# LanaSina/evolutionary_illusion_generator

Measured on AMD Instinct MI355X. Metric: genome fitness evals/sec at 256x256, pop=256, higher is better.
Workload: dtype f32; 1 GPU; neat_configs/circles.txt colour pop=256, 256x256, PredNet 3,48,96,192, 21 steps, LK + rotation-symmetry score; global_pop=256, genomes_per_gpu=256, device_batch=256, structure=Circles

## Files before the change

### evolutionary_illusion_generator_amd/csrc/conv_wino4.h

```cpp
#pragma once
#include "wino_launch.h"

namespace eig {

constexpr int W4_UPOS = 256;
constexpr int W4_U_FLOATS = W4_NPOS * W4_UPOS;
constexpr int W4_NUS = 3, W4_NPS = 3;
constexpr int w4_row(bool tall) { return tall ? 28 : 40; }
constexpr int w4_ps(bool tall) { return tall ? 1024 : 768; }
constexpr int w4_pslot(bool tall) { return W4_KC * w4_ps(tall); }
constexpr int w4_p(bool tall, int k) { return tall ? k * w4_pslot(true) : (k < 2 ? k * w4_pslot(false) : 2 * w4_pslot(false) + 3 * W4_U_FLOATS); }
constexpr int w4_u(bool tall, int k) { return tall ? 3 * w4_pslot(true) + k * W4_U_FLOATS : 2 * w4_pslot(false) + k * W4_U_FLOATS; }
constexpr int w4_x(bool tall) { return tall ? w4_u(true, 0) : w4_u(false, 1); }
constexpr int W4_X_FLOATS = W4_WAVES * 2 * 4 * 64 * 4;
constexpr int wino4_lds_bytes() { return (w4_x(false) + W4_X_FLOATS) * 4; }
static_assert((w4_u(true, 2) + W4_U_FLOATS) * 4 == wino4_lds_bytes() && (w4_p(false, 2) + w4_pslot(false)) * 4 <= wino4_lds_bytes(), "LDS maps");
#ifndef EIG_W4_DEEPU
#define EIG_W4_DEEPU 1
#endif
#ifndef EIG_W4_DIAG
#define EIG_W4_DIAG 0
#endif

__device__ __forceinline__ void w4_in1d(float d0, float d1, float d2, float d3, float d4, float d5, float* T)
{
    T[0] = fmaf(4.0f, d0, fmaf(-5.0f, d2, d4));
    const float p = fmaf(-4.0f, d2, d4), q = fmaf(-4.0f, d1, d3);
    T[1] = p + q; T[2] = p - q;
    const float r = d4 - d2, s = d3 - d1;
    T[3] = fmaf(2.0f, s, r); T[4] = fmaf(-2.0f, s, r);
    T[5] = fmaf(4.0f, d1, fmaf(-5.0f, d3, d5));
}
template <int XI> __device__ __forceinline__ float w4_row(const float* d)
{
    if constexpr (XI == 0) return fmaf(4.0f, d[0], fmaf(-5.0f, d[1], d[2]));
    else if constexpr (XI == 5) return fmaf(4.0f, d[0], fmaf(-5.0f, d[1], d[2]));
    else {
        if constexpr (XI == 1) return fmaf(-4.0f, d[1], d[3]) + fmaf(-4.0f, d[0], d[2]);
        else if constexpr (XI == 2) return fmaf(-4.0f, d[1], d[3]) - fmaf(-4.0f, d[0], d[2]);
        else if constexpr (XI == 3) return fmaf(2.0f, d[2] - d[0], d[3] - d[1]);
        else return fmaf(-2.0f, d[2] - d[0], d[3] - d[1]);
    }
}
constexpr int w4_nrows(int xi) { return (xi == 0 || xi == 5) ? 3 : 4; }
constexpr int w4_rowidx(int xi, int k) { return xi == 0 ? 2 * k : xi == 5 ? 2 * k + 1 : k + 1; }
constexpr int w4_uprow(int i) { return (i + 1) >> 1; }

template <typename V4> __device__ __forceinline__ void w4_out1d(const V4& m0, const V4& m1, const V4& m2, const V4& m3, const V4& m4, const V4& m5, V4* Y)
{
    const V4 s = m1 + m2, d = m1 - m2, u = m3 + m4, w = m3 - m4;
    Y[0] = (m0 + s) + u;
    for (int e = 0; e < 4; ++e) { Y[1][e] = fmaf(2.0f, w[e], d[e]); Y[2][e] = fmaf(4.0f, u[e], s[e]); Y[3][e] = fmaf(8.0f, w[e], d[e]) + m5[e]; }
}

template <int NI, int EPI, bool TALL = false, bool HALF = false, bool PACK = false, bool NSPLIT = false>
__global__ void __launch_bounds__((HALF && !NSPLIT) ? W4_THREADS / 2 : W4_THREADS, 3) wino4_kernel(const ConvArgs a)
{
    static_assert(!NSPLIT || (HALF && NI == 4 && EPI != EPI_CONVA), "N-split: a half block, 64-column N-blocks, ConvLSTM / ConvP");
    constexpr int NIW = NSPLIT ? 2 : NI;
    constexpr bool DEEPU = HALF && EIG_W4_DEEPU;
    static_assert(!(TALL && HALF), "half blocks exist in the wide shape only");
    static_assert(!PACK || (HALF && EPI != EPI_CONVA), "packed tiles: a half block, ConvLSTM / ConvP");
    constexpr bool TGEO = TALL || PACK;
    static_assert(EPI == EPI_LSTM || EPI == EPI_CONVA || EPI == EPI_CONVP, "conv_wino4.h: ConvLSTM, ConvA, ConvP");
    static_assert(EPI != EPI_LSTM || NI == 4, "ConvLSTM: the four N-tiles are the four gates");
    static_assert(NI == 3 || NI == 4, "N-blocks of 48 or 64 columns");
    constexpr int U4 = wino4_u_floats(NI);
    constexpr int KC = W4_KC, PS = w4_ps(TGEO), W4_ROW = w4_row(TGEO);
    constexpr int W4_P0 = w4_p(TGEO, 0), W4_P1 = w4_p(TGEO, 1), W4_P2 = w4_p(TGEO, 2), W4_U0 = w4_u(TGEO, 0), W4_U1 = w4_u(TGEO, 1), W4_U2 = w4_u(TGEO, 2);
    constexpr int PK_ROWS = 18, PK_CX = 7, PK_IMG = PK_ROWS * PK_CX;
    constexpr bool WALK = !TALL && !HALF;
    constexpr int RGH = TALL ? 16 : 8;
    extern __shared__ __attribute__((aligned(16))) float lds[];
    unsigned long long tq_entry = EIG_TIMING ? __builtin_readcyclecounter() : 0;
    float* const Pb = lds;
    float* const Ub = lds;
    float* const xb = lds + w4_x(TGEO);
    const int wv_o = __builtin_amdgcn_readfirstlane((int)threadIdx.x >> 6);
    const int rg_o = HALF ? 0 : wv_o & 1, xi_o = (HALF && !NSPLIT) ? wv_o : wv_o >> 1;
    const int ng_o = NSPLIT ? wv_o & 1 : 0;
    constexpr int NWAVES = (HALF && !NSPLIT) ? W4_WAVES / 2 : W4_WAVES;
    constexpr int UPW = 36 / NWAVES;
    auto lane_id = [&]() __attribute__((always_inline)) { int l = (int)__builtin_amdgcn_mbcnt_hi(~0u, __builtin_amdgcn_mbcnt_lo(~0u, 0u)); asm volatile("" : "+v"(l)); return l; };

    const int tiles = a.tilesX * a.tilesY;
    const bool pk5 = PACK && a.tilesX == 5;
    const int ntile = PACK ? a.B + (pk5 ? (a.B + 3) >> 2 : 0) : a.B * tiles;
    const int xcd = blockIdx.x & 7, xi_ = blockIdx.x >> 3;
    auto dv = [&](int x, int d, unsigned m) __attribute__((always_inline)) { return m ? (int)__umulhi((unsigned)x, m) : x / d; };
    const int q0 = dv(xi_, a.nparts, a.mg[0]);
    const int part = xi_ - q0 * a.nparts;
    const int tlin = a.tile_map ? xcd * ((ntile + 7) >> 3) + q0 : q0 * 8 + xcd;
    if (tlin >= ntile) return;
    const int nwalk = WALK ? a.nwalk : 1, nb0 = part * nwalk;
    const bool pk_edge_o = pk5 && tlin >= a.B;
    const int eb = PACK ? (pk_edge_o ? 4 * (tlin - a.B) : tlin) : dv(tlin, tiles, a.mg[1]);
    const int t_ = PACK ? 0 : tlin - eb * tiles;
    const int tyi = dv(t_, a.tilesX, a.mg[2]), txi = t_ - tyi * a.tilesX;
    const int y0 = PACK ? 0 : tyi * (TALL ? 32 : (HALF ? 8 : 16)), x0 = PACK ? 0 : txi * (TALL ? 16 : 32);
    const int HW = a.H * a.W;

    const bool up_fused = !PACK && EPI == EPI_LSTM && a.up_src != nullptr;
    const int nkb0 = a.src[0].C / KC;
    const int nkbu = up_fused ? (a.up_C / KC) : 0;
    const bool has1 = a.nsrc > 1;
    const int nkb_o = nkb0 + nkbu + (has1 ? (a.src[1].C / KC) : 0);
    const int up_lo_o = nkb0, up_hi_o = nkb0 + nkbu;
#define EIG4_WAITCNT(imm) do { __builtin_amdgcn_s_waitcnt(imm); asm volatile("" ::: "memory"); } while (0)
#define EIG4_BARRIER() do { asm volatile("" ::: "memory"); __builtin_amdgcn_s_barrier(); asm volatile("" ::: "memory"); } while (0)
#define EIG4_LDS_BARRIER() do { EIG4_WAITCNT(0xC07F); EIG4_BARRIER(); } while (0)
#define EIG4_IS_UP(kb) ((kb) >= up_lo && (kb) < up_hi)

    typedef float f32x2 __attribute__((ext_vector_type(2)));
    constexpr unsigned W4_POSB = 4 * 16 * NI * 4;
    auto walk_body = [&](const int it) __attribute__((always_inline)) {
    const int nblk = nb0 + it;
    int zs = 0;
    asm volatile("" : "+s"(zs));
    const int wv = wv_o + zs, rg = rg_o + zs, xi = xi_o + zs, ng = ng_o + zs, nkb = nkb_o + zs, up_lo = up_lo_o + zs, up_hi = up_hi_o + zs;
    const int pch = HALF ? wv >> 1 : wv / 3, ppart = HALF ? wv & 1 : wv - pch * 3;
    const bool has_plane = !(NSPLIT && !PACK) || wv_o < 8;
    const int eb_i = eb + zs, y0_i = y0 + zs, x0_i = x0 + zs;
    const bool pk_edge = (pk_edge_o ? 1 : 0) + zs != 0;
    const unsigned long long sb0 = (unsigned long long)(a.src[0].ptr + (size_t)eb_i * a.src[0].Ct * HW);
    const unsigned long long sb1 = has1 ? (unsigned long long)(a.src[1].ptr + (size_t)eb_i * a.src[1].Ct * HW) : sb0;
    const int ist0 = a.src[0].Ct * HW * 4, ist1 = has1 ? a.src[1].Ct * HW * 4 : ist0;
    const int sz0 = a.src[0].C * HW * 4 + (PACK ? 3 * ist0 : 0), sz1 = has1 ? a.src[1].C * HW * 4 + (PACK ? 3 * ist1 : 0) : sz0;
    const int Hh = a.H >> 1, Wh = a.W >> 1, HWh = Hh * Wh;
    const unsigned long long sbu = up_fused ? (unsigned long long)(a.up_src + (size_t)eb_i * a.up_C * HWh) : sb0;
    const int szu = up_fused ? a.up_C * HWh * 4 : sz0;
    const int lane = lane_id();
    const int q = lane >> 4, col = lane & 15;
    constexpr int CPR = TALL ? 7 : 10, CREAL = TALL ? 6 : 10, NCHK = TALL ? 34 * 7 : (HALF ? 100 : 180), UROWS = TALL ? 18 : (HALF ? 6 : 10), UCHK = TALL ? 4 : 6;
    auto plane_offsets = [&](int part, int& ro, int& uo) __attribute__((always_inline)) {
        const int c = lane + 64 * part;
        const int row = c / CPR, cx = c - row * CPR;
        const int gy = y0_i - 1 + row, gx = x0_i - 4 + 4 * cx;
        ro = (c < NCHK && cx < CREAL && gy >= 0 && gy < a.H && gx >= 0 && gx < a.W) ? (gy * a.W + gx) * 4 : -1;
        const int hy = (y0_i >> 1) - 1 + row, hx = (x0_i >> 1) - 4 + 4 * cx;
        uo = (row < UROWS && cx < UCHK && hy >= 0 && hy < Hh && hx >= 0 && hx < Wh) ? (hy * Wh + hx) * 4 : -1;
    };
    int pk_ro[3] = {-1, -1, -1};
    unsigned pk_mul[3] = {0u, 0u, 0u};
    const int pk_n = (wv_o < 4 ? 2 : 1) + (NSPLIT ? 0 : 1);
    if constexpr (PACK) {
#pragma unroll
        for (int k = 0; k < 3; ++k) {
            const int c = lane + 64 * ((wv_o + NWAVES * k) & 3);
            const int p = c >= PK_IMG ? 1 : 0, c1 = c - PK_IMG * p;
            const int row = c1 / PK_CX, slot = c1 - row * PK_CX;
            const int b = slot >= 3 ? (slot >= 6 ? 2 : 1) : 0;
            const int irel = pk_edge ? 2 * p + b : 0, cx = pk_edge ? 4 + slot - 3 * b : slot;
            const int gy = row - 1, gx = 4 * cx - 4;
            const bool ok = (pk_edge ? (c < 2 * PK_IMG && b < 2) : c < PK_IMG) && eb_i + irel < a.B && gy >= 0 && gy < a.H && gx >= 0 && gx < a.W;
            pk_ro[k] = ok ? (gy * a.W + gx) * 4 : -1;
            pk_mul[k] = ok ? (unsigned)irel : 0u;
        }
    }
    int roff, uoff, roff2 = -1, uoff2 = -1;
    plane_offsets(ppart, roff, uoff);
    const bool two_parts = (TALL && wv_o < 4) || (HALF && !PACK && !NSPLIT && wv_o < 2);
    if (TALL) plane_offsets(3, roff2, uoff2);
    if (HALF) { roff2 = roff; uoff2 = uoff; }
    const int ch2 = HALF ? 3 : wv, part2 = HALF ? ppart : 3;
    auto dma_plane_at = [&](int jj, int slot_off) __attribute__((always_inline)) {
        const int j = jj < nkb ? jj : nkb - 1;
        const bool up = EIG4_IS_UP(j);
        const bool s1 = j >= up_hi;
        const unsigned long long mu = 0ull - (unsigned long long)up, m1 = 0ull - (unsigned long long)s1;
        const unsigned long long u = sb0 + ((sb1 - sb0) & m1) + ((sbu - sb0) & mu);
        const unsigned lo = __builtin_amdgcn_readfirstlane((unsigned)u), hi = __builtin_amdgcn_readfirstlane((unsigned)(u >> 32));
        const int sz = sz0 + ((sz1 - sz0) & (int)m1) + ((szu - sz0) & (int)mu);
        const __amdgpu_buffer_rsrc_t rs = __builtin_amdgcn_make_buffer_rsrc((void*)(((unsigned long long)hi << 32) | lo), 0, __builtin_amdgcn_readfirstlane(sz), 0x00020000);
        const int base = (up_lo & (int)mu) + (up_hi & (int)m1), hw = HW + ((HWh - HW) & (int)mu);
        if constexpr (PACK) {
            const unsigned ist = (unsigned)(ist0 + ((ist1 - ist0) & (int)m1));
#pragma unroll
            for (int k = 0; k < 3; ++k) {
                if (k >= pk_n) break;
                const int idx = wv_o + NWAVES * k;
                const unsigned coffk = (unsigned)((j - base) * KC + (idx >> 2)) * (unsigned)(hw * 4);
                __builtin_amdgcn_raw_ptr_buffer_load_lds(rs, (__attribute__((address_space(3))) void*)(Pb + slot_off + (idx >> 2) * PS + (idx & 3) * 256), 16,
                                                         (int)__builtin_elementwise_add_sat((unsigned)pk_ro[k] + pk_mul[k] * ist, coffk), 0, 0, 0);
            }
            return;
        }
        if (!has_plane) return;
        const unsigned coff = (unsigned)((j - base) * KC + pch) * (unsigned)(hw * 4);
        __builtin_amdgcn_raw_ptr_buffer_load_lds(rs, (__attribute__((address_space(3))) void*)(Pb + slot_off + pch * PS + ppart * 256), 16,
                                                 (int)__builtin_elementwise_add_sat((unsigned)roff + (((unsigned)uoff - (unsigned)roff) & (unsigned)mu), coff), 0, 0, 0);
        if (two_parts) {
            const unsigned coff2 = (unsigned)((j - base) * KC + ch2) * (unsigned)(hw * 4);
            __builtin_amdgcn_raw_ptr_buffer_load_lds(rs, (__attribute__((address_space(3))) void*)(Pb + slot_off + ch2 * PS + part2 * 256), 16,
                                                     (int)__builtin_elementwise_add_sat((unsigned)roff2 + (((unsigned)uoff2 - (unsigned)roff2) & (unsigned)mu), coff2), 0, 0, 0);
        }
    };
    auto wait_u = [&]() __attribute__((always_inline)) {
        const int npl = PACK ? pk_n : (two_parts ? 2 : (has_plane ? 1 : 0));
        switch (npl + (DEEPU ? UPW : 0)) {
            case 0: EIG4_WAITCNT(0x0F70); break;
            case 1: EIG4_WAITCNT(0x0F71); break;
            case 2: EIG4_WAITCNT(0x0F72); break;
            case 3: EIG4_WAITCNT(0x0F73); break;
            case 4: EIG4_WAITCNT(0x0F74); break;
            case 5: EIG4_WAITCNT(0x0F75); break;
            case 6: EIG4_WAITCNT(0x0F76); break;
            case 7: EIG4_WAITCNT(0x0F77); break;
            case 8: EIG4_WAITCNT(0x0F78); break;
            default: EIG4_WAITCNT(0x0F79); break;
        }
    };
    const int uvo = (NI == 4 || lane < 48) ? lane * 16 : -1;
    auto prologue_a = [&](int nb) __attribute__((always_inline)) {
        const __amdgpu_buffer_rsrc_t rs = __builtin_amdgcn_make_buffer_rsrc((void*)(a.wpk + (size_t)nb * nkb * U4), 0, (nkb + 1) * U4 * 4, 0x00020000);
#pragma unroll
        for (int i = 0; i < UPW; ++i)
            __builtin_amdgcn_raw_ptr_buffer_load_lds(rs, (__attribute__((address_space(3))) void*)(Ub + W4_U0 + (UPW * wv + i) * W4_UPOS), 16, uvo, (int)((unsigned)(UPW * wv + i) * W4_POSB), 0, 0);
        dma_plane_at(0, W4_P0);
        dma_plane_at(1, W4_P1);
    };
    auto prologue_b = [&](int nb) __attribute__((always_inline)) {
        const __amdgpu_buffer_rsrc_t rs = __builtin_amdgcn_make_buffer_rsrc((void*)(a.wpk + (size_t)nb * nkb * U4), 0, (nkb + 1) * U4 * 4, 0x00020000);
#pragma unroll
        for (int i = 0; i < UPW; ++i)
            __builtin_amdgcn_raw_ptr_buffer_load_lds(rs, (__attribute__((address_space(3))) void*)(Ub + W4_U1 + (UPW * wv + i) * W4_UPOS), 16, uvo,
                                                     (int)((unsigned)U4 * 4 + (unsigned)(UPW * wv + i) * W4_POSB), 0, 0);
        dma_plane_at(2, W4_P2);
    };

    const int pk_ir = pk_edge ? col >> 2 : 0, pk_ty = pk_edge ? col & 3 : col >> 2;
    const int t_ty = PACK ? 0 : (TALL ? col >> 2 : col >> 3), t_tx = PACK ? (pk_edge ? 3 * (pk_ir & 1) : col & 3) : (TALL ? col & 3 : col & 7);
    const int pk_row = PACK ? PK_ROWS * (pk_ir >> 1) + 4 * pk_ty : 0;
    const float* const pbase_n = Pb + q * PS + (RGH * rg + 4 * t_ty + pk_row) * W4_ROW + 4 * t_tx;
    const float* const pbase_u = Pb + q * PS + ((RGH / 2) * rg + 2 * t_ty) * W4_ROW + 2 * t_tx + 3;
    const int b_off = xi * 6 * W4_UPOS + (q * 16 + col) * NI + 2 * ng;

    unsigned long long tq_setup = tq_entry;
    if (it == 0) {
        if (EIG_TIMING) tq_setup = __builtin_readcyclecounter();
        prologue_a(nb0);
        EIG4_WAITCNT(0x0F70);
    }
    const __amdgpu_buffer_rsrc_t rsw = __builtin_amdgcn_make_buffer_rsrc((void*)(a.wpk + (size_t)nblk * nkb * U4), 0, (nkb + 1) * U4 * 4, 0x00020000);
    unsigned u_so = (unsigned)(UPW * wv) * W4_POSB + 2u * (unsigned)U4 * 4u;
    auto dma_u = [&](int slot_off) __attribute__((always_inline)) {
#pragma unroll
        for (int i = 0; i < UPW; ++i)
            __builtin_amdgcn_raw_ptr_buffer_load_lds(rsw, (__attribute__((address_space(3))) void*)(Ub + slot_off + (UPW * wv + i) * W4_UPOS), 16, uvo,
                                                     (int)(u_so + (unsigned)i * W4_POSB), 0, 0);
        u_so += (unsigned)U4 * 4;
    };
    f32x4 acc[6][NIW];
#pragma unroll
    for (int p = 0; p < 6; ++p)
#pragma unroll
        for (int ni = 0; ni < NIW; ++ni) acc[p][ni] = (f32x4){0.f, 0.f, 0.f, 0.f};
    EIG4_BARRIER();
    prologue_b(nblk);
    const unsigned long long tq_k0 = EIG_TIMING ? __builtin_readcyclecounter() : 0;
    unsigned long long tq_k1 = 0, tq_x = 0, tq_y = 0;
    auto timeline = [&]() __attribute__((always_inline)) {
        if (EIG_TIMING && a.dbg && lane_id() == 0) {
            unsigned hwid, xcc;
            asm volatile("s_getreg_b32 %0, hwreg(HW_REG_HW_ID)" : "=s"(hwid));
            asm volatile("s_getreg_b32 %0, hwreg(HW_REG_XCC_ID)" : "=s"(xcc));
            unsigned long long* dd = a.dbg + (((size_t)blockIdx.x * nwalk + it) * NWAVES + wv) * 8;
            const unsigned long long tq_end = __builtin_readcyclecounter();
            dd[0] = tq_entry; dd[1] = tq_setup; dd[2] = tq_k0; dd[3] = tq_k1; dd[4] = tq_x; dd[5] = tq_y; dd[6] = tq_end;
            dd[7] = (unsigned long long)hwid | ((unsigned long long)xcc << 32);
            tq_entry = tq_end;
        }
    };

    auto kloops = [&](auto role_tag) __attribute__((always_inline)) {
        constexpr int XI = decltype(role_tag)::value;
        float v[6];
        float bq[NIW];
        int uo0 = W4_U0, uo1 = W4_U1, uo2 = W4_U2;
        int po0 = W4_P0, po1 = W4_P1, po2 = W4_P2;
        int pj = 0, psz = 0, pbound = 0;
// ... 131 lines not shown
                    if constexpr (!FIRST) read_b(uo1, 0, bq);
                    build_cols();
                }
            } else {
#pragma unroll
                for (int i = 0; i < NCH; ++i) {
                    const int nu = (UP && i >= 2) ? i + 1 : i;
                    if (i + 1 < NCH) {
                        const int nu1 = (UP && i + 1 >= 2) ? i + 2 : i + 1;
                        read_b(uo0, nu1, bv[(i + 1) & 1]);
                    } else if constexpr (!LAST && !FIRST) read_b(uo1, 0, bq);
                    const float* const b = i == 0 ? bq : bv[i & 1];
#pragma unroll
                    for (int ni = 0; ni < NIW; ++ni) acc[nu][ni] = __builtin_amdgcn_mfma_f32_16x16x4f32(v[nu], b[ni], acc[nu][ni], 0, 0, 0);
                    slice(i);
                    __builtin_amdgcn_sched_barrier(0);
                }
            }
            { const int t0 = uo0; uo0 = uo1; uo1 = uo2; uo2 = t0; }
            { const int t0 = po0; po0 = po1; po1 = po2; po2 = t0; }
            if (LAST || (EIG_W4_DIAG & (8 | 16))) EIG4_WAITCNT(0x0F70);
            else if (!(EIG_W4_DIAG & 2)) { if (!(EIG_W4_DIAG & 1)) wait_u(); }
            if (!(EIG_W4_DIAG & 2) || LAST) EIG4_BARRIER();
            if constexpr (FIRST) read_b(uo0, 0, bq);
        };
        const std::false_type nl{};
        const std::integral_constant<int, 2> rt{};
        int kb = 0;
        rows_begin(W4_P0, EIG4_IS_UP(0)); rows_mid(); rows_end();
        read_b(W4_U0, 0, bq);
        build_cols();
        EIG4_WAITCNT(0xC07F);
        EIG4_BARRIER();
        auto run = [&](const int end, auto kind_tag) __attribute__((always_inline)) {
            for (; kb + 1 < end; ++kb) kiter(kb, kind_tag, kind_tag, nl, nl);
            if (kb + 1 == end && end < nkb) { kiter(kb, kind_tag, rt, nl, nl); ++kb; }
        };
        kiter(0, std::integral_constant<int, 0>{}, std::integral_constant<int, 0>{}, nl, std::true_type{});
        kb = 1;
        run(up_lo, std::integral_constant<int, 0>{});
        run(up_hi, std::integral_constant<int, 1>{});
        run(nkb, std::integral_constant<int, 0>{});
        kiter(nkb - 1, rt, rt, std::true_type{}, nl);
    };
    switch (xi) {
        case 0: kloops(std::integral_constant<int, 0>{}); break;
        case 1: kloops(std::integral_constant<int, 1>{}); break;
        case 2: kloops(std::integral_constant<int, 2>{}); break;
        case 3: kloops(std::integral_constant<int, 3>{}); break;
        case 4: kloops(std::integral_constant<int, 4>{}); break;
        default: kloops(std::integral_constant<int, 5>{}); break;
    }
    if (EIG_TIMING) tq_k1 = __builtin_readcyclecounter();
    const bool more = it + 1 < nwalk;
    if (more) prologue_a(nblk + 1);

    f32x4 cc[4][NIW];
#pragma unroll
    for (int ni = 0; ni < NIW; ++ni) {
        f32x4 Y[4];
        w4_out1d(acc[0][ni], acc[1][ni], acc[2][ni], acc[3][ni], acc[4][ni], acc[5][ni], Y);
#pragma unroll
        for (int b = 0; b < 4; ++b) cc[b][ni] = Y[b];
    }
    {
    int zf = 0;
    asm volatile("" : "+s"(zf));
    const int eb = eb_i + zf, y0 = y0_i + zf, x0 = x0_i + zf, wv = wv_o + zf, rg = rg_o + zf, xi = xi_o + zf, HWf = HW + zf, Cout = a.Cout + zf, ngf = ng_o + zf;
    const bool pk_edge_f = (pk_edge_o ? 1 : 0) + zf != 0;
    const int lane = lane_id();
    const int q = lane >> 4, col = lane & 15;
    const size_t cHW = (size_t)HWf;
    const int j = TALL ? lane & 3 : lane & 7, chl = TALL ? lane >> 2 : lane >> 3, e_r = j & 3, ql = TALL ? 0 : j >> 2;
    int woff[4];
#pragma unroll
    for (int e = 0; e < 4; ++e) woff[e] = (((2 * xi + (NSPLIT ? ngf : rg)) * 2 * 4 + e) * 64 + q * 16 + ((col + 4 * e + (PACK ? q : (TALL ? 0 : 8 * (q & 1)))) & 15)) * 4;
    const int fr = lane & 15, fchl = lane >> 4;
    const int f_i = pk_edge_f ? fr >> 2 : 0, f_ty = pk_edge_f ? fr & 3 : fr >> 2, f_tx = pk_edge_f ? 4 : fr & 3;
    if constexpr (EPI == EPI_LSTM || EPI == EPI_CONVP) {
        const int nun = NSPLIT ? ((xi < 4 && ngf == 0) ? 2 : 1) : (xi < 4 ? 3 : 2);
        auto unit_cq = [&](int un) __attribute__((always_inline)) { return xi < 4 ? (NSPLIT ? (ngf ? 2 : un) : un) : 3; };
        auto unit_arow = [&](int un) __attribute__((always_inline)) { return xi < 4 ? xi : 2 * (xi - 4) + (NSPLIT ? ngf : un); };
        int xoff[3];
#pragma unroll
        for (int un = 0; un < 3; ++un) {
            const int cq = unit_cq(un);
            const int ty = TALL ? cq : cq >> 1, chh = TALL ? 0 : cq & 1;
            xoff[un] = TALL ? (e_r * 64 + ty * 16 + ((chl + 4 * e_r) & 15)) * 4 : (e_r * 64 + (2 * ty + ql) * 16 + ((8 * chh + chl + 4 * e_r + 8 * ql) & 15)) * 4;
            if constexpr (PACK) xoff[un] = ((fr & 3) * 64 + (fr >> 2) * 16 + ((4 * cq + fchl + 4 * (fr & 3) + (fr >> 2)) & 15)) * 4;
        }
        auto finish = [&](int arow, int nr, int off, int xw) __attribute__((always_inline)) -> f32x4 {
            auto C = [&](int x) __attribute__((always_inline)) { return *reinterpret_cast<const f32x4*>(xb + ((x * 2 + xw) * 2 + nr) * 1024 + off); };
            const f32x4 c1 = C(1), c2 = C(2), c3 = C(3), c4 = C(4);
            const f32x4 s_ = c1 + c2, d_ = c1 - c2, u_ = c3 + c4, w_ = c3 - c4;
            f32x4 y;
            if (arow == 0) { const f32x4 c0 = C(0); y = (c0 + s_) + u_; }
            else if (arow == 1) { for (int b = 0; b < 4; ++b) y[b] = fmaf(2.0f, w_[b], d_[b]); }
            else if (arow == 2) { for (int b = 0; b < 4; ++b) y[b] = fmaf(4.0f, u_[b], s_[b]); }
            else { const f32x4 c5 = C(5); for (int b = 0; b < 4; ++b) y[b] = fmaf(8.0f, w_[b], d_[b]) + c5[b]; }
            return y;
        };
        f32x4 ys[NI][3];
        auto finish_unit = [&](int ni, int nr, int xw, int un) __attribute__((always_inline)) {
            const int sel = NSPLIT ? ngf : un;
            switch (xi) {
                case 0: ys[ni][un] = finish(0, nr, xoff[un], xw); break;
                case 1: ys[ni][un] = finish(1, nr, xoff[un], xw); break;
                case 2: ys[ni][un] = finish(2, nr, xoff[un], xw); break;
                case 3: ys[ni][un] = finish(3, nr, xoff[un], xw); break;
                case 4: ys[ni][un] = sel ? finish(1, nr, xoff[un], xw) : finish(0, nr, xoff[un], xw); break;
                default: ys[ni][un] = sel ? finish(3, nr, xoff[un], xw) : finish(2, nr, xoff[un], xw); break;
            }
        };
        if constexpr (NSPLIT) {
#pragma unroll
            for (int nr = 0; nr < 2; ++nr)
#pragma unroll
                for (int e = 0; e < 4; ++e) {
                    f32x4 t;
                    t[0] = cc[0][nr][e]; t[1] = cc[1][nr][e]; t[2] = cc[2][nr][e]; t[3] = cc[3][nr][e];
                    *reinterpret_cast<f32x4*>(xb + woff[e] + nr * 1024) = t;
                }
            EIG4_LDS_BARRIER();
            if (EIG_TIMING) tq_x = __builtin_readcyclecounter();
#pragma unroll
            for (int ni = 0; ni < NI; ++ni)
#pragma unroll
                for (int un = 0; un < 2; ++un) {
                    if (un >= nun) break;
                    finish_unit(ni, ni & 1, ni >> 1, un);
                }
        } else {
#pragma unroll
        for (int rnd = 0; rnd < 2; ++rnd) {
            if (2 * rnd >= NI) break;
            if (rnd) EIG4_LDS_BARRIER();
#pragma unroll
            for (int nr = 0; nr < 2; ++nr) {
                const int ni = 2 * rnd + nr;
                if (ni >= NI) break;
#pragma unroll
                for (int e = 0; e < 4; ++e) {
                    f32x4 t;
                    t[0] = cc[0][ni][e]; t[1] = cc[1][ni][e]; t[2] = cc[2][ni][e]; t[3] = cc[3][ni][e];
                    *reinterpret_cast<f32x4*>(xb + woff[e] + nr * 1024) = t;
                }
            }
            EIG4_LDS_BARRIER();
            if (EIG_TIMING && rnd == 0) tq_x = __builtin_readcyclecounter();
#pragma unroll
            for (int nr = 0; nr < 2; ++nr) {
                const int ni = 2 * rnd + nr;
                if (ni >= NI) break;
#pragma unroll
                for (int un = 0; un < 3; ++un) {
                    if (un >= nun) break;
                    finish_unit(ni, nr, rg, un);
                }
            }
        }
        }
        if (more) EIG4_WAITCNT(0x0F70);
        if (EIG_TIMING) { asm volatile("s_waitcnt lgkmcnt(0)" ::: "memory"); tq_y = __builtin_readcyclecounter(); }
#pragma unroll
        for (int un = 0; un < 3; ++un) {
            if (un >= nun) break;
            const int cq = unit_cq(un);
            const int ty = TALL ? cq : cq >> 1, chh = TALL ? 0 : cq & 1;
            const int arow = unit_arow(un);
            const int gy = PACK ? 4 * f_ty + arow : y0 + RGH * rg + 4 * ty + arow, gx = PACK ? 4 * f_tx : x0 + 4 * j;
            if (gy >= a.H || gx >= a.W) continue;
            const int ebo = PACK ? eb + f_i : eb;
            if (PACK && ebo >= a.B) continue;
            const size_t pix = (size_t)gy * a.W + gx;
            const int chq = PACK ? 4 * cq + fchl : 8 * chh + chl;
            if constexpr (EPI == EPI_LSTM) {
                const int ch = nblk * 16 + chq;
                if (ch >= Cout) continue;
                const float bi = a.bias[ch], bf = a.bias[Cout + ch], bc = a.bias[2 * Cout + ch], bo = a.bias[3 * Cout + ch];
                const size_t cbase = ((size_t)ebo * Cout + ch) * cHW, ps = (size_t)Cout * cHW, pbase = (size_t)ch * cHW;
                const f32x4 cold4 = *reinterpret_cast<const f32x4*>(a.c_state + cbase + pix);
                const f32x4 pi4 = *reinterpret_cast<const f32x4*>(a.peep + pbase + pix);
                const f32x4 pf4 = *reinterpret_cast<const f32x4*>(a.peep + ps + pbase + pix);
                const f32x4 po4 = *reinterpret_cast<const f32x4*>(a.peep + 2 * ps + pbase + pix);
                f32x4 cn4, hn4;
#pragma unroll
                for (int b = 0; b < 4; ++b) {
                    float cn, hn;
                    lstm_cell(ys[0][un][b], ys[1][un][b], ys[2][un][b], ys[3][un][b], bi, bf, bc, bo, cold4[b], pi4[b], pf4[b], po4[b], cn, hn);
                    cn4[b] = cn; hn4[b] = hn;
                }
                *reinterpret_cast<f32x4*>(a.c_state + cbase + pix) = cn4;
                *reinterpret_cast<f32x4*>(a.h_out + cbase + pix) = hn4;
            } else {
#pragma unroll
                for (int ni = 0; ni < NI; ++ni) {
                    const int ch = (nblk * NI + ni) * 16 + chq;
                    if (ch >= Cout) continue;
                    const float bb_ = a.bias[ch];
                    f32x4 v4;
#pragma unroll
                    for (int b = 0; b < 4; ++b) v4[b] = relu_f(ys[ni][un][b] + bb_);
                    *reinterpret_cast<f32x4*>(a.Pout + ((size_t)ebo * Cout + ch) * cHW + pix) = v4;
                }
            }
        }
    } else {
        const int Ho = a.H >> 1, Wo = a.W >> 1;
        const size_t plane = (size_t)Ho * Wo;
        const int ox = (x0 >> 1) + 2 * j;
#pragma unroll
// ... 10 lines not shown
                    f32x4 t;
                    t[0] = cc[0][ni][e]; t[1] = cc[1][ni][e]; t[2] = cc[2][ni][e]; t[3] = cc[3][ni][e];
                    *reinterpret_cast<f32x4*>(xb + woff[e] + nr * 1024) = t;
                }
            }
            EIG4_LDS_BARRIER();
            if (rnd == (NI - 1) / 2) { if (more) EIG4_WAITCNT(0x0F70); }
            if (EIG_TIMING && rnd == 0) { tq_x = __builtin_readcyclecounter(); tq_y = tq_x; }
            const int g0 = nval == 2 ? (xi < 4 ? 3 * xi : 12 + 2 * (xi - 4)) : (xi < 2 ? 2 * xi : xi + 2);
            const int cnt = nval == 2 ? (xi < 4 ? 3 : 2) : (xi < 2 ? 2 : 1);
#pragma unroll
            for (int un = 0; un < 3; ++un) {
                if (un >= cnt) break;
                const int g = g0 + un;
                const int nr = g >> 3, ty = TALL ? (g >> 1) & 3 : (g >> 2) & 1, ap = TALL ? g & 1 : (g >> 1) & 1, chh = TALL ? 0 : g & 1;
                const int off = TALL ? ((nr + 2 * rg) * 256 + e_r * 64 + ty * 16 + ((chl + 4 * e_r) & 15)) * 4
                                     : ((nr + 2 * rg) * 256 + e_r * 64 + (2 * ty + ql) * 16 + ((8 * chh + chl + 4 * e_r + 8 * ql) & 15)) * 4;
                auto C = [&](int x) __attribute__((always_inline)) { return *reinterpret_cast<const f32x4*>(xb + x * 4096 + off); };
                const f32x4 c1 = C(1), c2 = C(2), c3 = C(3), c4 = C(4);
                const f32x4 s_ = c1 + c2, d_ = c1 - c2, u_ = c3 + c4, w_ = c3 - c4;
                f32x4 ya, yb;
                if (ap == 0) {
                    const f32x4 c0 = C(0);
                    ya = (c0 + s_) + u_;
                    for (int b = 0; b < 4; ++b) yb[b] = fmaf(2.0f, w_[b], d_[b]);
                } else {
                    const f32x4 c5 = C(5);
                    for (int b = 0; b < 4; ++b) { ya[b] = fmaf(4.0f, u_[b], s_[b]); yb[b] = fmaf(8.0f, w_[b], d_[b]) + c5[b]; }
                }
                const int ch = (nblk * NI + 2 * rnd + nr) * 16 + 8 * chh + chl;
                const int oy = (y0 >> 1) + (RGH / 2) * rg + 2 * ty + ap;
                if (oy >= Ho || ox >= Wo || ch >= Cout) continue;
                const float bb_ = a.bias[ch];
                const size_t pb = ((size_t)eb * Cout + ch) * plane + (size_t)oy * Wo + ox;
                const size_t e0 = ((size_t)eb * 2 * Cout + ch) * plane + (size_t)oy * Wo + ox, e1 = e0 + (size_t)Cout * plane;
                const f32x2 p2 = *reinterpret_cast<const f32x2*>(a.P + pb);
                f32x2 ea, eb2;
#pragma unroll
                for (int bp = 0; bp < 2; ++bp) {
                    const float v00 = relu_f(ya[2 * bp] + bb_), v01 = relu_f(ya[2 * bp + 1] + bb_);
                    const float v10 = relu_f(yb[2 * bp] + bb_), v11 = relu_f(yb[2 * bp + 1] + bb_);
                    const float A = fmaxf(fmaxf(v00, v01), fmaxf(v10, v11));
                    ea[bp] = relu_f(A - p2[bp]);
                    eb2[bp] = relu_f(p2[bp] - A);
                }
                *reinterpret_cast<f32x2*>(a.E + e0) = ea;
                *reinterpret_cast<f32x2*>(a.E + e1) = eb2;
            }
        }
    }
    }
    timeline();
    };
    for (int it = 0; it < nwalk; ++it) walk_body(it);
#undef EIG4_WAITCNT
#undef EIG4_BARRIER
#undef EIG4_LDS_BARRIER
#undef EIG4_IS_UP
}

}
```

### evolutionary_illusion_generator_amd/csrc/eigen_engine.hip

```cpp
#include <hip/hip_runtime.h>

#include <algorithm>
#include <cmath>
#include <cstdarg>
#include <cstdio>
#include <cstring>
#include <string>
#include <unordered_map>
#include <unordered_set>
#include <vector>

#include "../../include/eigen_engine.h"
#define EIG_ENGINE_UNIT 1
#include "conv_mfma.h"
#include "wino_launch.h"
#include "cppn_kernel.h"
#include "farneback_kernels.h"
#include "flow_kernels.h"
#include "score_kernels.h"

using namespace eig;

static thread_local std::string g_err;
static int fail(int code, const char* fmt, ...)
// ... 391 lines not shown
    }
}

static hipError_t launch_conv(eigen_engine* e, ConvOp& op, ConvArgs& a, int batch, hipStream_t st)
{
    const int TH = (op.TW == 8) ? 8 : 16;
    const int NIMG = 256 / (TH * op.TW);
    a.H = op.H; a.W = op.W; a.B = batch;
    a.tilesX = (op.W + op.TW - 1) / op.TW;
    a.tilesY = (op.H + TH - 1) / TH;
    a.n_nblk = op.n_nblk; a.krows = op.krows; a.wpk = op.d_wpk; a.Cout = op.Cout; a.zeros = e->d_zeros;
    a.nsrc = op.nsrc;
    for (int s = 0; s < op.nsrc; ++s) { a.src[s].C = op.src_C[s]; a.src[s].Cpad = pad4(op.src_C[s]); a.src[s]._reserved = 0; a.src[s].Ct = op.src_Ct[s] ? op.src_Ct[s] : op.src_C[s]; }
    int ntile = ((batch + NIMG - 1) / NIMG) * a.tilesX * a.tilesY;
    const int per_tile = op.n_nblk * (op.epi == EPI_UP4 ? 4 : 1);
    int grid = per_tile * ((ntile + 7) / 8) * 8;
    const bool vec = (op.W % 4) == 0;
#if EIG_TIMING
    unsigned long long* tl_dbg = nullptr;
    if (getenv("EIGEN_TIMELINE") && (op.epi == EPI_LSTM || (op.epi == EPI_UP4 && op.NI == 4) || (op.wino && getenv("EIGEN_TIMELINE_ALL"))) && ++op.tl_seen == 6) {
        (void)hipMalloc((void**)&tl_dbg, (size_t)grid * 2 * 64 * 8);
        (void)hipMemset(tl_dbg, 0, (size_t)grid * 2 * 64 * 8);
        a.dbg = tl_dbg;
    }
#endif
    {
        static const int tile_map = getenv("EIGEN_TILE_MAP") ? atoi(getenv("EIGEN_TILE_MAP")) : 1;
        a.tile_map = tile_map != 0;
    }
    static const int w8_env = getenv("EIGEN_W8") ? atoi(getenv("EIGEN_W8")) : -1;
    const int w8 = (vec && op.epi == EPI_CONVA && op.TW == 16 && op.NI < 4 && (w8_env >= 0 ? w8_env != 0 : grid <= 8 * e->n_cu)) ? 1 : 0;
    op.last_grid = grid; op.last_waves = (w8 == 1) ? 8 : 4;
    if (e->profile_convs) (void)hipEventRecord(e->pev0, st);
    hipError_t r;
    if (op.wino) {
        if (op.epi == EPI_LSTM && a.acc_init != nullptr) return hipErrorInvalidConfiguration;
        static const int tall_env = getenv("EIGEN_W4_TALL") ? atoi(getenv("EIGEN_W4_TALL")) : -1;
        const bool tall = tall_env >= 0 ? tall_env != 0 : ((op.W + 15) / 16) * ((op.H + 31) / 32) < ((op.W + 31) / 32) * ((op.H + 15) / 16);
        a.tilesX = tall ? (op.W + 15) / 16 : (op.W + 31) / 32; a.tilesY = tall ? (op.H + 31) / 32 : (op.H + 15) / 16;
        static const int half_env = getenv("EIGEN_W4_HALF") ? atoi(getenv("EIGEN_W4_HALF")) : -1;
        const bool half = !tall && (half_env >= 0 ? half_env != 0 : (long long)op.n_nblk * batch * a.tilesX * ((op.H + 7) / 8) <= e->n_cu);
        if (half) a.tilesY = (op.H + 7) / 8;
        static const int pack_env = getenv("EIGEN_W4_PACK") ? atoi(getenv("EIGEN_W4_PACK")) : -1;
        const int ptx = (op.W + 3) / 4, pty = (op.H + 3) / 4;
        const bool pack_can = op.epi != EPI_CONVA && a.up_src == nullptr && (ptx == 4 || ptx == 5) && pty == 4 && tall_env < 0 && half_env < 0;
        bool pack = false;
        if (pack_can) {
            const long long nhalf = (long long)op.n_nblk * (batch + (ptx == 5 ? (batch + 3) / 4 : 0)), nfull = (long long)op.n_nblk * batch;
            pack = pack_env >= 0 ? pack_env != 0 : 2 * ((nhalf + e->n_cu - 1) / e->n_cu) < 3 * ((nfull + e->n_cu - 1) / e->n_cu);
        }
        if (pack) { a.tilesX = ptx; a.tilesY = pty; }
        const int ntile4 = pack ? batch + (ptx == 5 ? (batch + 3) / 4 : 0) : batch * a.tilesX * a.tilesY;
        static const int parts_env = getenv("EIGEN_W4_PARTS") ? atoi(getenv("EIGEN_W4_PARTS")) : 0;
        int nparts;
        if (parts_env > 0) { nparts = std::min(parts_env, op.n_nblk); while (op.n_nblk % nparts) --nparts; }
        else {
            int nwalk = (op.n_nblk % 3 == 0) ? 3 : ((op.n_nblk % 2 == 0) ? 2 : 1);
            if ((long long)(op.n_nblk / nwalk) * ntile4 < 4ll * e->n_cu) nwalk = 1;
            nparts = op.n_nblk / nwalk;
        }
        if (tall || half || pack) nparts = op.n_nblk;
        a.nparts = nparts; a.nwalk = op.n_nblk / nparts;
        const int g4 = nparts * ((ntile4 + 7) / 8) * 8;
        {
            auto magic = [&](long long d) -> unsigned { return (d > 1 && (long long)g4 * 16 * d < (1ll << 32)) ? (unsigned)(((1ll << 32) + d - 1) / d) : 0u; };
            a.mg[0] = magic(nparts); a.mg[1] = magic((long long)a.tilesX * a.tilesY); a.mg[2] = magic(a.tilesX);
        }
        op.last_grid = g4 * a.nwalk; op.last_waves = ((half || pack) && !(op.NI == 4 && op.epi != EPI_CONVA)) ? W4_WAVES / 2 : W4_WAVES;
#if EIG_TIMING
        if (tl_dbg) {
            (void)hipFree(tl_dbg);
            (void)hipMalloc((void**)&tl_dbg, (size_t)op.last_grid * op.last_waves * 64);
            (void)hipMemset(tl_dbg, 0, (size_t)op.last_grid * op.last_waves * 64);
            a.dbg = tl_dbg;
        }
#endif
        r = launch_wino4(op.NI, op.epi, pack ? W4_PACK : (tall ? W4_TALL : (half ? W4_HALF : W4_WIDE)), a, g4, st);
    } else {
    static const bool direct_p0 = !(getenv("EIGEN_CONVP0_MFMA") && atoi(getenv("EIGEN_CONVP0_MFMA")));
    if (op.epi == EPI_CONVP && op.d_wraw && direct_p0) {
        const dim3 g((op.W + P0_TX - 1) / P0_TX, (op.H + P0_TY - 1) / P0_TY, batch);
        if (op.Cout == 3) hipLaunchKernelGGL(convp0_direct_kernel<3>, g, dim3(P0_TX * P0_TY), 0, st, a.src[0].ptr, op.d_wraw, a);
        else hipLaunchKernelGGL(convp0_direct_kernel<1>, g, dim3(P0_TX * P0_TY), 0, st, a.src[0].ptr, op.d_wraw, a);
        r = hipGetLastError();
    } else if (static const bool direct_l0 = !(getenv("EIGEN_LSTM0_MFMA") && atoi(getenv("EIGEN_LSTM0_MFMA")));
               op.epi == EPI_LSTM_PACKED && op.d_wraw && direct_l0 && (op.Cout == 1 || op.Cout == 3)) {
        const dim3 g((op.W + L0_TX - 1) / L0_TX, (op.H + L0_TY - 1) / L0_TY, batch);
        const dim3 blk(L0_TX * L0_TY);
        const float *sE = a.src[0].ptr, *sH = a.src[1].ptr;
        if (op.nsrc == 1) {
            if (op.Cout == 3) hipLaunchKernelGGL((lstm0_direct_kernel<3, true>), g, blk, 0, st, sE, sH, op.d_wraw, a);
            else hipLaunchKernelGGL((lstm0_direct_kernel<1, true>), g, blk, 0, st, sE, sH, op.d_wraw, a);
        } else {
            if (op.Cout == 3) hipLaunchKernelGGL((lstm0_direct_kernel<3, false>), g, blk, 0, st, sE, sH, op.d_wraw, a);
            else hipLaunchKernelGGL((lstm0_direct_kernel<1, false>), g, blk, 0, st, sE, sH, op.d_wraw, a);
        }
        r = hipGetLastError();
    } else
    switch (op.epi) {
        case EPI_LSTM: r = (op.TW == 16) ? launch_inst<4, 16, EPI_LSTM>(a, grid, st, vec) : launch_inst<4, 8, EPI_LSTM>(a, grid, st, vec); break;
        case EPI_LSTM_PACKED: r = (op.TW == 16) ? launch_inst<1, 16, EPI_LSTM_PACKED>(a, grid, st, vec) : launch_inst<1, 8, EPI_LSTM_PACKED>(a, grid, st, vec); break;
        case EPI_CONVA: {
            static const bool onekb = !(getenv("EIGEN_NO_ONEKB") && atoi(getenv("EIGEN_NO_ONEKB")));
            if (onekb && op.NI == 3 && op.TW == 16 && vec && op.nsrc == 1 && pad4(op.src_C[0]) <= KC) r = launch_inst2<3, 16, EPI_CONVA, true, true>(a, grid, st);
            else r = launch_epi<EPI_CONVA>(op.NI, op.TW, a, grid, st, vec, w8);
            break;
        }
        case EPI_CONVP: r = launch_epi<EPI_CONVP>(op.NI, op.TW, a, grid, st, vec, w8); break;
        case EPI_UP4: r = launch_epi<EPI_UP4>(op.NI, op.TW, a, grid, st, vec, w8); break;
        case EPI_UP4C: r = launch_inst2<4, 16, EPI_UP4C, true>(a, grid, st); break;
        default: r = launch_epi<EPI_RAW>(op.NI, op.TW, a, grid, st, vec, w8); break;
    }
    }
#if EIG_TIMING
    if (tl_dbg) {
        (void)hipStreamSynchronize(st);
        std::vector<unsigned long long> h((size_t)op.last_grid * op.last_waves * 8);
        (void)hipMemcpy(h.data(), tl_dbg, h.size() * 8, hipMemcpyDeviceToHost);
        char name[256];
// ... 1133 lines not shown
```

Before: 429.1 genome evals/s.

## Let Winograd conv blocks walk across tile boundaries with tuned walk length

For non-LSTM wide Winograd convs, each block now walks a flattened sequence of (tile, N-block) work items instead of only the N-blocks of one tile. The walk length is picked by a host-side score that balances rounds per XCD against walk length. When a walk crosses into the next tile, the kernel prefetches that tile's input plane and weights. This aims to balance load across CUs and amortise prologue latency, at the cost of more index arithmetic and kernarg reloads inside the loop.

After: 428.6 genome evals/s (median of 2 runs). Within noise of the previous version (-0.1%).

```diff
diff --git a/evolutionary_illusion_generator_amd/csrc/conv_wino4.h b/evolutionary_illusion_generator_amd/csrc/conv_wino4.h
--- a/evolutionary_illusion_generator_amd/csrc/conv_wino4.h
+++ b/evolutionary_illusion_generator_amd/csrc/conv_wino4.h
@@ -70,6 +70,7 @@
     constexpr int W4_P0 = w4_p(TGEO, 0), W4_P1 = w4_p(TGEO, 1), W4_P2 = w4_p(TGEO, 2), W4_U0 = w4_u(TGEO, 0), W4_U1 = w4_u(TGEO, 1), W4_U2 = w4_u(TGEO, 2);
     constexpr int PK_ROWS = 18, PK_CX = 7, PK_IMG = PK_ROWS * PK_CX;
     constexpr bool WALK = !TALL && !HALF;
+    constexpr bool XWALK = WALK && EPI != EPI_LSTM;
     constexpr int RGH = TALL ? 16 : 8;
     extern __shared__ __attribute__((aligned(16))) float lds[];
     unsigned long long tq_entry = EIG_TIMING ? __builtin_readcyclecounter() : 0;
@@ -88,16 +89,27 @@
     const int ntile = PACK ? a.B + (pk5 ? (a.B + 3) >> 2 : 0) : a.B * tiles;
     const int xcd = blockIdx.x & 7, xi_ = blockIdx.x >> 3;
     auto dv = [&](int x, int d, unsigned m) __attribute__((always_inline)) { return m ? (int)__umulhi((unsigned)x, m) : x / d; };
-    const int q0 = dv(xi_, a.nparts, a.mg[0]);
-    const int part = xi_ - q0 * a.nparts;
+    const int q0 = XWALK ? dv(xi_ * a.nwalk, a.n_nblk, a.mg[0]) : dv(xi_, a.nparts, a.mg[0]);
+    const int part = XWALK ? xi_ * a.nwalk - q0 * a.n_nblk : xi_ - q0 * a.nparts;
     const int tlin = a.tile_map ? xcd * ((ntile + 7) >> 3) + q0 : q0 * 8 + xcd;
     if (tlin >= ntile) return;
-    const int nwalk = WALK ? a.nwalk : 1, nb0 = part * nwalk;
+    const int nwalk = WALK ? a.nwalk : 1, nb0 = XWALK ? part : part * nwalk;
+    const int xtiles = a.tile_map ? min((ntile + 7) >> 3, ntile - xcd * ((ntile + 7) >> 3)) : (ntile - xcd + 7) >> 3;
+    const int nw = XWALK ? min(nwalk, xtiles * a.n_nblk - xi_ * nwalk) : nwalk;
     const bool pk_edge_o = pk5 && tlin >= a.B;
     const int eb = PACK ? (pk_edge_o ? 4 * (tlin - a.B) : tlin) : dv(tlin, tiles, a.mg[1]);
     const int t_ = PACK ? 0 : tlin - eb * tiles;
     const int tyi = dv(t_, a.tilesX, a.mg[2]), txi = t_ - tyi * a.tilesX;
     const int y0 = PACK ? 0 : tyi * (TALL ? 32 : (HALF ? 8 : 16)), x0 = PACK ? 0 : txi * (TALL ? 16 : 32);
+    typedef const __attribute__((address_space(4))) ConvArgs* karg_ptr;
+    auto ka = [&]() __attribute__((always_inline)) { karg_ptr p = (karg_ptr)__builtin_amdgcn_kernarg_segment_ptr(); asm volatile("" : "+s"(p)); return p; };
+    auto tile_at = [&](int tl, int& e, int& yy, int& xx) __attribute__((always_inline)) {
+        const karg_ptr k = ka();
+        const int tX = k->tilesX;
+        e = dv(tl, tX * k->tilesY, k->mg[1]);
+        const int tt = tl - e * (tX * k->tilesY), ty = dv(tt, tX, k->mg[2]);
+        yy = ty * 16; xx = (tt - ty * tX) * 32;
+    };
     const int HW = a.H * a.W;
 
     const bool up_fused = !PACK && EPI == EPI_LSTM && a.up_src != nullptr;
@@ -114,13 +126,24 @@
     typedef float f32x2 __attribute__((ext_vector_type(2)));
     constexpr unsigned W4_POSB = 4 * 16 * NI * 4;
     auto walk_body = [&](const int it) __attribute__((always_inline)) {
-    const int nblk = nb0 + it;
+    int nblk = nb0 + it;
+    int eb_w = eb, y0_w = y0, x0_w = x0, tl_w = tlin;
+    if constexpr (XWALK) {
+        int zw = 0;
+        asm volatile("" : "+s"(zw));
+        const karg_ptr k = ka();
+        const int nbz = nblk + zw;
+        const int dt = dv(nbz, k->n_nblk, k->mg[0]);
+        nblk = nbz - dt * k->n_nblk;
+        tl_w = tlin + zw + dt * (k->tile_map ? 1 : 8);
+        tile_at(tl_w, eb_w, y0_w, x0_w);
+    }
     int zs = 0;
     asm volatile("" : "+s"(zs));
     const int wv = wv_o + zs, rg = rg_o + zs, xi = xi_o + zs, ng = ng_o + zs, nkb = nkb_o + zs, up_lo = up_lo_o + zs, up_hi = up_hi_o + zs;
     const int pch = HALF ? wv >> 1 : wv / 3, ppart = HALF ? wv & 1 : wv - pch * 3;
     const bool has_plane = !(NSPLIT && !PACK) || wv_o < 8;
-    const int eb_i = eb + zs, y0_i = y0 + zs, x0_i = x0 + zs;
+    const int eb_i = eb_w + zs, y0_i = y0_w + zs, x0_i = x0_w + zs;
     const bool pk_edge = (pk_edge_o ? 1 : 0) + zs != 0;
     const unsigned long long sb0 = (unsigned long long)(a.src[0].ptr + (size_t)eb_i * a.src[0].Ct * HW);
     const unsigned long long sb1 = has1 ? (unsigned long long)(a.src[1].ptr + (size_t)eb_i * a.src[1].Ct * HW) : sb0;
@@ -132,14 +155,15 @@
     const int lane = lane_id();
     const int q = lane >> 4, col = lane & 15;
     constexpr int CPR = TALL ? 7 : 10, CREAL = TALL ? 6 : 10, NCHK = TALL ? 34 * 7 : (HALF ? 100 : 180), UROWS = TALL ? 18 : (HALF ? 6 : 10), UCHK = TALL ? 4 : 6;
-    auto plane_offsets = [&](int part, int& ro, int& uo) __attribute__((always_inline)) {
+    auto plane_offsets_at = [&](int part, int ty0, int tx0, int& ro, int& uo) __attribute__((always_inline)) {
         const int c = lane + 64 * part;
         const int row = c / CPR, cx = c - row * CPR;
-        const int gy = y0_i - 1 + row, gx = x0_i - 4 + 4 * cx;
+        const int gy = ty0 - 1 + row, gx = tx0 - 4 + 4 * cx;
         ro = (c < NCHK && cx < CREAL && gy >= 0 && gy < a.H && gx >= 0 && gx < a.W) ? (gy * a.W + gx) * 4 : -1;
-        const int hy = (y0_i >> 1) - 1 + row, hx = (x0_i >> 1) - 4 + 4 * cx;
+        const int hy = (ty0 >> 1) - 1 + row, hx = (tx0 >> 1) - 4 + 4 * cx;
         uo = (row < UROWS && cx < UCHK && hy >= 0 && hy < Hh && hx >= 0 && hx < Wh) ? (hy * Wh + hx) * 4 : -1;
     };
+    auto plane_offsets = [&](int part, int& ro, int& uo) __attribute__((always_inline)) { plane_offsets_at(part, y0_i, x0_i, ro, uo); };
     int pk_ro[3] = {-1, -1, -1};
     unsigned pk_mul[3] = {0u, 0u, 0u};
     const int pk_n = (wv_o < 4 ? 2 : 1) + (NSPLIT ? 0 : 1);
@@ -211,11 +235,14 @@
         }
     };
     const int uvo = (NI == 4 || lane < 48) ? lane * 16 : -1;
-    auto prologue_a = [&](int nb) __attribute__((always_inline)) {
+    auto prologue_a_u = [&](int nb) __attribute__((always_inline)) {
         const __amdgpu_buffer_rsrc_t rs = __builtin_amdgcn_make_buffer_rsrc((void*)(a.wpk + (size_t)nb * nkb * U4), 0, (nkb + 1) * U4 * 4, 0x00020000);
 #pragma unroll
         for (int i = 0; i < UPW; ++i)
             __builtin_amdgcn_raw_ptr_buffer_load_lds(rs, (__attribute__((address_space(3))) void*)(Ub + W4_U0 + (UPW * wv + i) * W4_UPOS), 16, uvo, (int)((unsigned)(UPW * wv + i) * W4_POSB), 0, 0);
+    };
+    auto prologue_a = [&](int nb) __attribute__((always_inline)) {
+        prologue_a_u(nb);
         dma_plane_at(0, W4_P0);
         dma_plane_at(1, W4_P1);
     };
@@ -226,6 +253,20 @@
             __builtin_amdgcn_raw_ptr_buffer_load_lds(rs, (__attribute__((address_space(3))) void*)(Ub + W4_U1 + (UPW * wv + i) * W4_UPOS), 16, uvo,
                                                      (int)((unsigned)U4 * 4 + (unsigned)(UPW * wv + i) * W4_POSB), 0, 0);
         dma_plane_at(2, W4_P2);
+    };
+    auto prologue_a_tile = [&](int tl) __attribute__((always_inline)) {
+        int ebn, y0n, x0n, ron, uon, zt = 0;
+        asm volatile("" : "+s"(zt));
+        tile_at(tl + zt, ebn, y0n, x0n);
+        prologue_a_u(0);
+        plane_offsets_at(ppart, y0n, x0n, ron, uon);
+        const unsigned long long u = (unsigned long long)(a.src[0].ptr + (size_t)ebn * a.src[0].Ct * HW);
+        const unsigned lo = __builtin_amdgcn_readfirstlane((unsigned)u), hi = __builtin_amdgcn_readfirstlane((unsigned)(u >> 32));
+        const __amdgpu_buffer_rsrc_t rs = __builtin_amdgcn_make_buffer_rsrc((void*)(((unsigned long long)hi << 32) | lo), 0, __builtin_amdgcn_readfirstlane(sz0), 0x00020000);
+#pragma unroll
+        for (int j = 0; j < 2; ++j)
+            __builtin_amdgcn_raw_ptr_buffer_load_lds(rs, (__attribute__((address_space(3))) void*)(Pb + (j ? W4_P1 : W4_P0) + pch * PS + ppart * 256), 16,
+                                                     (int)__builtin_elementwise_add_sat((unsigned)ron, (unsigned)(j * KC + pch) * (unsigned)(HW * 4)), 0, 0, 0);
     };
 
     const int pk_ir = pk_edge ? col >> 2 : 0, pk_ty = pk_edge ? col & 3 : col >> 2;
@@ -463,8 +504,14 @@
         default: kloops(std::integral_constant<int, 5>{}); break;
     }
     if (EIG_TIMING) tq_k1 = __builtin_readcyclecounter();
-    const bool more = it + 1 < nwalk;
-    if (more) prologue_a(nblk + 1);
+    const bool more = it + 1 < nw;
+    if (more) {
+        if constexpr (XWALK) {
+            const karg_ptr k = ka();
+            if (nblk + 1 < k->n_nblk) prologue_a(nblk + 1);
+            else prologue_a_tile(tl_w + (k->tile_map ? 1 : 8));
+        } else prologue_a(nblk + 1);
+    }
 
     f32x4 cc[4][NIW];
 #pragma unroll
@@ -684,7 +731,7 @@
     }
     timeline();
     };
-    for (int it = 0; it < nwalk; ++it) walk_body(it);
+    for (int it = 0; it < nw; ++it) walk_body(it);
 #undef EIG4_WAITCNT
 #undef EIG4_BARRIER
 #undef EIG4_LDS_BARRIER
diff --git a/evolutionary_illusion_generator_amd/csrc/eigen_engine.hip b/evolutionary_illusion_generator_amd/csrc/eigen_engine.hip
--- a/evolutionary_illusion_generator_amd/csrc/eigen_engine.hip
+++ b/evolutionary_illusion_generator_amd/csrc/eigen_engine.hip
@@ -467,19 +467,31 @@
         if (pack) { a.tilesX = ptx; a.tilesY = pty; }
         const int ntile4 = pack ? batch + (ptx == 5 ? (batch + 3) / 4 : 0) : batch * a.tilesX * a.tilesY;
         static const int parts_env = getenv("EIGEN_W4_PARTS") ? atoi(getenv("EIGEN_W4_PARTS")) : 0;
-        int nparts;
-        if (parts_env > 0) { nparts = std::min(parts_env, op.n_nblk); while (op.n_nblk % nparts) --nparts; }
-        else {
-            int nwalk = (op.n_nblk % 3 == 0) ? 3 : ((op.n_nblk % 2 == 0) ? 2 : 1);
+        static const int walk_max = getenv("EIGEN_W4_WALK_MAX") ? std::max(1, atoi(getenv("EIGEN_W4_WALK_MAX"))) : 8;
+        const bool xwalk = op.epi != EPI_LSTM && !(tall || half || pack);
+        const long long xtiles = (ntile4 + 7) / 8, xitems = xtiles * op.n_nblk, xcus = std::max(1, e->n_cu / 8);
+        int nparts, nwalk;
+        if (parts_env > 0) { nparts = std::min(parts_env, op.n_nblk); while (op.n_nblk % nparts) --nparts; nwalk = op.n_nblk / nparts; }
+        else if (xwalk) {
+            nwalk = 1;
+            long long best = -1;
+            for (int w = 1; w <= walk_max; ++w) {
+                const long long rounds = ((xitems + w - 1) / w + xcus - 1) / xcus, score = rounds * w * 4 - (w % op.n_nblk == 0 ? 2 : 0);
+                if (best < 0 || score <= best) { best = score; nwalk = w; }
+            }
+            nparts = std::max(1, op.n_nblk / nwalk);
+        } else {
+            nwalk = (op.n_nblk % 3 == 0) ? 3 : ((op.n_nblk % 2 == 0) ? 2 : 1);
             if ((long long)(op.n_nblk / nwalk) * ntile4 < 4ll * e->n_cu) nwalk = 1;
             nparts = op.n_nblk / nwalk;
         }
-        if (tall || half || pack) nparts = op.n_nblk;
-        a.nparts = nparts; a.nwalk = op.n_nblk / nparts;
-        const int g4 = nparts * ((ntile4 + 7) / 8) * 8;
+        if (tall || half || pack) { nparts = op.n_nblk; nwalk = 1; }
+        a.nparts = nparts; a.nwalk = nwalk;
+        const int g4 = xwalk ? (int)((xitems + nwalk - 1) / nwalk) * 8 : nparts * ((ntile4 + 7) / 8) * 8;
         {
-            auto magic = [&](long long d) -> unsigned { return (d > 1 && (long long)g4 * 16 * d < (1ll << 32)) ? (unsigned)(((1ll << 32) + d - 1) / d) : 0u; };
-            a.mg[0] = magic(nparts); a.mg[1] = magic((long long)a.tilesX * a.tilesY); a.mg[2] = magic(a.tilesX);
+            const long long xmax = xwalk ? 8 * (xitems + nwalk) : g4;
+            auto magic = [&](long long d) -> unsigned { return (d > 1 && xmax * 16 * d < (1ll << 32)) ? (unsigned)(((1ll << 32) + d - 1) / d) : 0u; };
+            a.mg[0] = magic(xwalk ? op.n_nblk : nparts); a.mg[1] = magic((long long)a.tilesX * a.tilesY); a.mg[2] = magic(a.tilesX);
         }
         op.last_grid = g4 * a.nwalk; op.last_waves = ((half || pack) && !(op.NI == 4 && op.epi != EPI_CONVA)) ? W4_WAVES / 2 : W4_WAVES;
 #if EIG_TIMING
```

## Remap epilogue units so each lane finishes multiple output rows sharing LDS reads

Applied to the files above, without the earlier changes.

Swaps the role of xi and unit index in the Winograd F(4,3) epilogue: units now map to channel-quads and output rows, so one lane computes several output rows of the same tile column. A templated finish_rows helper loads the shared transform columns c1..c4 once and derives consecutive output rows from them, instead of reloading them for each row. This removes redundant LDS reads and runtime switch dispatch. It also adds an FDIAG diagnostic mode, off by default, that replaces LDS reads with synthetic values.

Result: no change. 427.9 genome evals/s before, 431.3 genome evals/s after, median of 6 (+0.8%).

```diff
diff --git a/evolutionary_illusion_generator_amd/csrc/conv_wino4.h b/evolutionary_illusion_generator_amd/csrc/conv_wino4.h
--- a/evolutionary_illusion_generator_amd/csrc/conv_wino4.h
+++ b/evolutionary_illusion_generator_amd/csrc/conv_wino4.h
@@ -20,6 +20,9 @@
 #endif
 #ifndef EIG_W4_DIAG
 #define EIG_W4_DIAG 0
+#endif
+#ifndef EIG_W4_FDIAG
+#define EIG_W4_FDIAG 0
 #endif
 
 __device__ __forceinline__ void w4_in1d(float d0, float d1, float d2, float d3, float d4, float d5, float* T)
@@ -490,8 +493,8 @@
     const int f_i = pk_edge_f ? fr >> 2 : 0, f_ty = pk_edge_f ? fr & 3 : fr >> 2, f_tx = pk_edge_f ? 4 : fr & 3;
     if constexpr (EPI == EPI_LSTM || EPI == EPI_CONVP) {
         const int nun = NSPLIT ? ((xi < 4 && ngf == 0) ? 2 : 1) : (xi < 4 ? 3 : 2);
-        auto unit_cq = [&](int un) __attribute__((always_inline)) { return xi < 4 ? (NSPLIT ? (ngf ? 2 : un) : un) : 3; };
-        auto unit_arow = [&](int un) __attribute__((always_inline)) { return xi < 4 ? xi : 2 * (xi - 4) + (NSPLIT ? ngf : un); };
+        auto unit_cq = [&](int un) __attribute__((always_inline)) { return xi < 4 ? xi : 2 * (xi - 4) + (NSPLIT ? ngf : un); };
+        auto unit_arow = [&](int un) __attribute__((always_inline)) { return xi < 4 ? (NSPLIT ? (ngf ? 2 : un) : un) : 3; };
         int xoff[3];
 #pragma unroll
         for (int un = 0; un < 3; ++un) {
@@ -500,27 +503,29 @@
             xoff[un] = TALL ? (e_r * 64 + ty * 16 + ((chl + 4 * e_r) & 15)) * 4 : (e_r * 64 + (2 * ty + ql) * 16 + ((8 * chh + chl + 4 * e_r + 8 * ql) & 15)) * 4;
             if constexpr (PACK) xoff[un] = ((fr & 3) * 64 + (fr >> 2) * 16 + ((4 * cq + fchl + 4 * (fr & 3) + (fr >> 2)) & 15)) * 4;
         }
-        auto finish = [&](int arow, int nr, int off, int xw) __attribute__((always_inline)) -> f32x4 {
-            auto C = [&](int x) __attribute__((always_inline)) { return *reinterpret_cast<const f32x4*>(xb + ((x * 2 + xw) * 2 + nr) * 1024 + off); };
+        auto finish_rows = [&](auto r0_tag, auto nr_tag, int nr, int off, int xw, f32x4* y) __attribute__((always_inline)) {
+            constexpr int R0 = decltype(r0_tag)::value, R1 = R0 + decltype(nr_tag)::value - 1;
+            auto C = [&](int x) __attribute__((always_inline)) -> f32x4 {
+                if constexpr ((EIG_W4_FDIAG & 1) != 0) { const float f = __int_as_float(off + x + nr + xw); return (f32x4){f, f, f, f}; }
+                else return *reinterpret_cast<const f32x4*>(xb + ((x * 2 + xw) * 2 + nr) * 1024 + off);
+            };
             const f32x4 c1 = C(1), c2 = C(2), c3 = C(3), c4 = C(4);
             const f32x4 s_ = c1 + c2, d_ = c1 - c2, u_ = c3 + c4, w_ = c3 - c4;
-            f32x4 y;
-            if (arow == 0) { const f32x4 c0 = C(0); y = (c0 + s_) + u_; }
-            else if (arow == 1) { for (int b = 0; b < 4; ++b) y[b] = fmaf(2.0f, w_[b], d_[b]); }
-            else if (arow == 2) { for (int b = 0; b < 4; ++b) y[b] = fmaf(4.0f, u_[b], s_[b]); }
-            else { const f32x4 c5 = C(5); for (int b = 0; b < 4; ++b) y[b] = fmaf(8.0f, w_[b], d_[b]) + c5[b]; }
-            return y;
+            if constexpr (R0 == 0) { const f32x4 c0 = C(0); y[0] = (c0 + s_) + u_; }
+            if constexpr (R0 <= 1 && R1 >= 1) { for (int b = 0; b < 4; ++b) y[1 - R0][b] = fmaf(2.0f, w_[b], d_[b]); }
+            if constexpr (R0 <= 2 && R1 >= 2) { for (int b = 0; b < 4; ++b) y[2 - R0][b] = fmaf(4.0f, u_[b], s_[b]); }
+            if constexpr (R1 == 3) { const f32x4 c5 = C(5); for (int b = 0; b < 4; ++b) y[3 - R0][b] = fmaf(8.0f, w_[b], d_[b]) + c5[b]; }
         };
         f32x4 ys[NI][3];
-        auto finish_unit = [&](int ni, int nr, int xw, int un) __attribute__((always_inline)) {
-            const int sel = NSPLIT ? ngf : un;
-            switch (xi) {
-                case 0: ys[ni][un] = finish(0, nr, xoff[un], xw); break;
-                case 1: ys[ni][un] = finish(1, nr, xoff[un], xw); break;
-                case 2: ys[ni][un] = finish(2, nr, xoff[un], xw); break;
-                case 3: ys[ni][un] = finish(3, nr, xoff[un], xw); break;
-                case 4: ys[ni][un] = sel ? finish(1, nr, xoff[un], xw) : finish(0, nr, xoff[un], xw); break;
-                default: ys[ni][un] = sel ? finish(3, nr, xoff[un], xw) : finish(2, nr, xoff[un], xw); break;
+        auto finish_units = [&](int ni, int nr, int xw) __attribute__((always_inline)) {
+            using std::integral_constant;
+            if (xi < 4) {
+                if constexpr (!NSPLIT) finish_rows(integral_constant<int, 0>{}, integral_constant<int, 3>{}, nr, xoff[0], xw, &ys[ni][0]);
+                else if (ngf == 0) finish_rows(integral_constant<int, 0>{}, integral_constant<int, 2>{}, nr, xoff[0], xw, &ys[ni][0]);
+                else finish_rows(integral_constant<int, 2>{}, integral_constant<int, 1>{}, nr, xoff[0], xw, &ys[ni][0]);
+            } else {
+#pragma unroll
+                for (int un = 0; un < (NSPLIT ? 1 : 2); ++un) finish_rows(integral_constant<int, 3>{}, integral_constant<int, 1>{}, nr, xoff[un], xw, &ys[ni][un]);
             }
         };
         if constexpr (NSPLIT) {
@@ -535,12 +540,7 @@
             EIG4_LDS_BARRIER();
             if (EIG_TIMING) tq_x = __builtin_readcyclecounter();
 #pragma unroll
-            for (int ni = 0; ni < NI; ++ni)
-#pragma unroll
-                for (int un = 0; un < 2; ++un) {
-                    if (un >= nun) break;
-                    finish_unit(ni, ni & 1, ni >> 1, un);
-                }
+            for (int ni = 0; ni < NI; ++ni) finish_units(ni, ni & 1, ni >> 1);
         } else {
 #pragma unroll
         for (int rnd = 0; rnd < 2; ++rnd) {
@@ -563,11 +563,7 @@
             for (int nr = 0; nr < 2; ++nr) {
                 const int ni = 2 * rnd + nr;
                 if (ni >= NI) break;
-#pragma unroll
-                for (int un = 0; un < 3; ++un) {
-                    if (un >= nun) break;
-                    finish_unit(ni, nr, rg, un);
-                }
+                finish_units(ni, nr, rg);
             }
         }
         }
```
